# redradman/MujocoPoseLearning

Hardware: AMD Instinct MI355X
Metric: env steps/sec (whole node), humanoid 'stand' task, 1/2/4/8 MI355X (higher is better)
Workload: dtype f64

## Files before the change

### mujocoposelearning_amd/csrc/hs_contacts.h

```cpp
#pragma once
#include "hs_lanes.h"
#include "hs_scratch.h"

namespace hs {
namespace {

template <typename T>
struct Con {
  T pos[3], n[3], t1[3], dist;
};

template <typename T>
__device__ __forceinline__ bool plane_sphere(const T* pp, const T* pn, const T* c, T r, Con<T>& o) {
  T d[3] = {c[0] - pp[0], c[1] - pp[1], c[2] - pp[2]};
  T cd = dot3(d, pn);
  if (cd > r) return false;
  o.dist = cd - r;
  for (int k = 0; k < 3; k++) { o.n[k] = pn[k]; o.pos[k] = c[k] - pn[k] * (o.dist * T(0.5) + r); o.t1[k] = 0; }
  return true;
}
template <typename T>
__device__ __forceinline__ bool sphere_sphere(const T* p1, T r1, const T* p2, T r2, Con<T>& o) {
  T d[3] = {p2[0] - p1[0], p2[1] - p1[1], p2[2] - p1[2]};
  T len = sqrt(dot3(d, d));
// ... 56 lines not shown
  } else {
    T ax1[3] = {a1[0] * h1, a1[1] * h1, a1[2] * h1}, ax2[3] = {a2[0] * h2, a2[1] * h2, a2[2] * h2};
    T dif[3] = {p1[0] - p2[0], p1[1] - p2[1], p1[2] - p2[2]};
    T ma = dot3(ax1, ax1), mb = -dot3(ax1, ax2), mc = dot3(ax2, ax2), u = -dot3(ax1, dif), v = dot3(ax2, dif);
    T det = ma * mc - mb * mb;
    T v1[3], v2[3];
    if (fabs(det) >= T(1e-15)) {
      T x1 = (mc * u - mb * v) / det, x2 = (ma * v - mb * u) / det;
      if (x1 > 1) { x1 = 1; x2 = (v - mb) / mc; }
      else if (x1 < -1) { x1 = -1; x2 = (v + mb) / mc; }
      if (x2 > 1) { x2 = 1; x1 = (u - mb) / ma; x1 = x1 > 1 ? 1 : (x1 < -1 ? -1 : x1); }
      else if (x2 < -1) { x2 = -1; x1 = (u + mb) / ma; x1 = x1 > 1 ? 1 : (x1 < -1 ? -1 : x1); }
      for (int k = 0; k < 3; k++) { v1[k] = p1[k] + x1 * ax1[k]; v2[k] = p2[k] + x2 * ax2[k]; }
      n = sphere_sphere(v1, r1, v2, r2, c0) ? 1 : 0;
    } else {
      for (int side = 1; side >= -1; side -= 2) {
        T x2 = (v - side * mb) / mc;
        x2 = x2 > 1 ? 1 : (x2 < -1 ? -1 : x2);
        for (int k = 0; k < 3; k++) { v1[k] = p1[k] + side * ax1[k]; v2[k] = p2[k] + x2 * ax2[k]; }
        Con<T> t;
        if (sphere_sphere(v1, r1, v2, r2, t)) { if (n == 0) c0 = t; else c1 = t; n++; }
      }
    }
  }
  if (n > 0) make_frame(c0);
  if (n > 1) make_frame(c1);
  return n;
}

template <typename T, typename C>
__device__ __forceinline__ void store_contact(MPtr<T> m, Scratch<T, C>& s, int slot, const Con<T>& c, int p) {
  if (slot >= C::CON) return;
  for (int k = 0; k < 3; k++) { s.con_pos[slot][k] = c.pos[k]; s.con_n[slot][k] = c.n[k]; s.con_t1[slot][k] = c.t1[k]; }
  s.con_dist[slot] = c.dist;
  s.con_pair[slot] = p;
  const int b1 = m->pair_b1[p], b2 = m->pair_b2[p];
  s.con_bb[slot] = (uint32_t)b1 | (uint32_t)b2 << 8 | (uint32_t)m->pair_dim[p] << 16;
  s.con_m1[slot] = b1 ? HS_LT(C, m).body_chainmask[b1] : 0u;
  s.con_m2[slot] = HS_LT(C, m).body_chainmask[b2];
  s.con_mu[slot] = m->pair_mu[p];
}

static_assert(MAXPAIR <= 256 && MAXGEOM <= 256 && PAIR_CAPSULE_CAPSULE < 256, "near-pair entry: one byte per field");
__device__ __forceinline__ uint32_t near_entry(int p, int g1, int g2, int fn) {
  return (uint32_t)p | (uint32_t)g1 << 8 | (uint32_t)g2 << 16 | (uint32_t)fn << 24;
}
template <typename T, typename C>
__device__ __forceinline__ void store_contact_near(MPtr<T> m, Scratch<T, C>& s, int slot, const Con<T>& c, int p,
                                                   int g1, int g2, int dim, T mu) {
  if (slot >= C::CON) return;
  for (int k = 0; k < 3; k++) { s.con_pos[slot][k] = c.pos[k]; s.con_n[slot][k] = c.n[k]; s.con_t1[slot][k] = c.t1[k]; }
  s.con_dist[slot] = c.dist;
  s.con_pair[slot] = p;
  const int b1 = lanes<C>(m).geom_bodyid[g1], b2 = lanes<C>(m).geom_bodyid[g2];
  s.con_bb[slot] = (uint32_t)b1 | (uint32_t)b2 << 8 | (uint32_t)dim << 16;
  s.con_m1[slot] = b1 ? lanes<C>(m).body_chainmask[b1] : 0u;
  s.con_m2[slot] = lanes<C>(m).body_chainmask[b2];
  s.con_mu[slot] = mu;
}

template <typename T>
__device__ __forceinline__ T impedance(CPtr<T> si, T pos, T margin) {
  T s0 = fmin(T(0.9999), fmax(T(0.0001), si[0])), s1 = fmin(T(0.9999), fmax(T(0.0001), si[1]));
  if (s0 == s1 || si[2] <= T(1e-15)) return T(0.5) * (s0 + s1);
  T x = (pos - margin) * si[5];
  if (x < 0) x = -x;
  if (x >= 1 || x <= 0) return x >= 1 ? s1 : s0;
  const T p = si[4];
  T y = x;
  if (p != T(1)) {
    const bool lo = x <= si[3];
    const T base = lo ? x : 1 - x;
    T pw = base * base;
    if (p != T(2)) pw = pow(base, p);
    y = lo ? pw * si[6] : 1 - pw * si[7];
  }
  return s0 + y * (s1 - s0);
}

template <typename C, typename T>
__device__ __forceinline__ uint32_t chain_mask(MPtr<T> m, int sl, int nb) {
  return (sl > 0 && sl < nb) ? HS_LT(C, m).body_chainmask[sl] : 0u;
}
template <int NV, typename T, typename C>
__device__ __forceinline__ void map_vx(Scratch<T, C>& s, int sl, int nb, uint32_t ch) {
  if (sl < nb) {
    T v[6] = {0, 0, 0, 0, 0, 0};
    HS_FOR_BITS(C, G_VX, T)(ch, [&](int j) { ValsX<T, 6> r; r.x = s.vx[j]; for (int k = 0; k < 6; k++) r.v[k] = s.cdof[j][k]; return r; },
                [&](int, const ValsX<T, 6>& r) {
#pragma unroll
                  for (int k = 0; k < 6; k++) v[k] = fma(r.v[k], r.x, v[k]);
                });
    for (int k = 0; k < 6; k++) s.u.n.bvel[sl][k] = v[k];
  }
  WSYNC();
#pragma unroll
  for (int cs = 0; cs < C::CON; cs += HL) {
    const int c = cs + sl;
    if (c < s.ncon) {
      const uint32_t bb = s.con_bb[c];
      const int b1 = bb & 0xff, b2 = (bb >> 8) & 0xff;
      T r[3] = {s.con_pos[c][0] - s.com[0], s.con_pos[c][1] - s.com[1], s.con_pos[c][2] - s.com[2]};
      T w[3], v1[3], v2[3];
      cross3(s.u.n.bvel[b2], r, w);
      for (int k = 0; k < 3; k++) v2[k] = s.u.n.bvel[b2][3 + k] + w[k];
      cross3(s.u.n.bvel[b1], r, w);
      for (int k = 0; k < 3; k++) v1[k] = s.u.n.bvel[b1][3 + k] + w[k];
      T dv[3] = {v2[0] - v1[0], v2[1] - v1[1], v2[2] - v1[2]};
      T t2[3];
      cross3(s.con_n[c], s.con_t1[c], t2);
      s.con_v[c][0] = dot3(s.con_n[c], dv);
      s.con_v[c][1] = dot3(s.con_t1[c], dv);
      s.con_v[c][2] = dot3(t2, dv);
    }
  }
  WSYNC();
}

template <typename T, typename C>
__device__ __forceinline__ T row_Jx(MPtr<T> m, const Scratch<T, C>& s, int desc, T coef) {
  int kind = rk_kind(desc), j = rk_id(desc);
  if (kind <= RK_JHI) return coef * s.vx[j];
  if (kind <= RK_THI) {
    T v = 0;
    for (int w = 0; w < HS_LT(C, m).ten_nwrap[j]; w++) v += HS_LT(C, m).ten_wrapcoef[j][w] * s.vx[HS_LT(C, m).ten_wrapdof[j][w]];
    return coef * v;
  }
  int comp = kind == RK_CN ? 1 : 1 + ((kind - RK_P0) >> 1);
  return s.con_v[j][0] + coef * s.con_v[j][comp];
}

template <typename T, typename C>
__device__ __forceinline__ void row_u(MPtr<T> m, const Scratch<T, C>& s, int kind, int c, T* u) {
  if (kind == RK_CN) { for (int k = 0; k < 3; k++) u[k] = s.con_n[c][k]; return; }
  int sub = kind - RK_P0;
  T mu = s.con_mu[c];
  T sg = (sub & 1) ? -mu : mu;
  T t[3];
  if (sub >> 1) cross3(s.con_n[c], s.con_t1[c], t);
  else { t[0] = s.con_t1[c][0]; t[1] = s.con_t1[c][1]; t[2] = s.con_t1[c][2]; }
  for (int k = 0; k < 3; k++) u[k] = s.con_n[c][k] + sg * t[k];
}

template <typename T, typename C>
__device__ __forceinline__ void contact_aggregates(MPtr<T> m, Scratch<T, C>& s, int sl) {
  const bool up = threadIdx.x >= HL;
#pragma unroll
  for (int cs = 0; cs < C::CON; cs += HL) {
    const int c = cs + sl;
    bool act = false;
    if (c < s.ncon) {
      int adr = s.con_adr[c];
      int nr = (s.con_bb[c] >> 16) == 1 ? 1 : 4;
      T U[6] = {0, 0, 0, 0, 0, 0}, F[3] = {0, 0, 0};
      const bool pyr = nr == 4;
      T f4[4], D4[4], nn[3], t1[3], t2[3];
#pragma unroll
      for (int q = 0; q < 4; q++) {
        const bool on = q == 0 || pyr;
        f4[q] = on ? s.row_f[adr + q] : T(0);
        D4[q] = on ? s.row_D[adr + q] : T(0);
      }
      for (int k = 0; k < 3; k++) { nn[k] = s.con_n[c][k]; t1[k] = s.con_t1[c][k]; }
      const T mu = s.con_mu[c];
      cross3(nn, t1, t2);
#pragma unroll
      for (int q = 0; q < 4; q++) {
        const T f = f4[q];
        if (f != T(0)) {
          T u[3];
          if (!pyr) {
            for (int k = 0; k < 3; k++) u[k] = nn[k];
          } else {
            const T sg = (q & 1) ? -mu : mu;
            for (int k = 0; k < 3; k++) u[k] = nn[k] + sg * ((q >> 1) ? t2[k] : t1[k]);
          }
          const T D = D4[q];
          U[0] += D * u[0] * u[0]; U[1] += D * u[1] * u[1]; U[2] += D * u[2] * u[2];
          U[3] += D * u[0] * u[1]; U[4] += D * u[0] * u[2]; U[5] += D * u[1] * u[2];
          for (int k = 0; k < 3; k++) F[k] += f * u[k];
        }
      }
      for (int k = 0; k < 6; k++) s.con_U[c][k] = U[k];
      for (int k = 0; k < 3; k++) s.con_F[c][k] = F[k];
      act = F[0] != T(0) || F[1] != T(0) || F[2] != T(0) || U[0] != T(0) || U[1] != T(0) || U[2] != T(0);
    }
    const uint32_t mk = hballot(act, up);
    if (sl == 0) s.con_act[cs / HL] = mk;
  }
  WSYNC();
}
template <typename C, typename F>
__device__ __forceinline__ void for_active_contacts(const uint32_t* act, F&& f) {
#pragma unroll
  for (int w = 0; w < (C::CON + HL - 1) / HL; w++)
    for (uint32_t mk = act[w]; mk; mk &= mk - 1u) f(w * HL + __builtin_ctz(mk));
}

template <typename T, typename C, typename LD, typename F>
__device__ __forceinline__ void for_active_contacts_ld(const uint32_t* act, LD&& ld, F&& f) {
#pragma unroll
  for (int w = 0; w < (C::CON + HL - 1) / HL; w++)
    for_bits<T, true>(
        act[w], [&](int j) { return ld(w * HL + j); }, [&](int j, const auto& v) { f(w * HL + j, v); });
}

template <typename T, typename C>
__device__ __forceinline__ T jtf_lane(MPtr<T> m, const Scratch<T, C>& s, int sl, const T* cd) {
  T acc = 0;
  struct CV { uint32_t m1, m2; T p[3], f[3]; };
  for_active_contacts_ld<T, C>(s.con_act, [&](int c) {
    CV v;
    v.m1 = s.con_m1[c]; v.m2 = s.con_m2[c];
    for (int k = 0; k < 3; k++) { v.p[k] = s.con_pos[c][k]; v.f[k] = s.con_F[c][k]; }
    return v;
  }, [&](int, const CV& v) {
    const int in2 = bit(v.m2, sl), in1 = bit(v.m1, sl);
    if (in1 != in2) {
      T r[3] = {v.p[0] - s.com[0], v.p[1] - s.com[1], v.p[2] - s.com[2]};
      T w[3];
      cross3(cd, r, w);
      T jp[3] = {cd[3] + w[0], cd[4] + w[1], cd[5] + w[2]};
      T x = dot3(jp, v.f);
      acc += in2 ? x : -x;
    }
  });
  if (sl < MAXDOF) {
    int lr = s.lim_row[sl];
    int lo = (lr & 0xff) - 1, hi = (lr >> 8) - 1;
    if (lo >= 0) acc += s.row_f[lo];
    if (hi >= 0) acc -= s.row_f[hi];
  }
  for (int r = s.njl; r < s.nlim; r++) {
    int id = rk_id(s.row_kid[r]);
    T f = rk_kind(s.row_kid[r]) == RK_TLO ? s.row_f[r] : -s.row_f[r];
    for (int w = 0; w < HS_LT(C, m).ten_nwrap[id]; w++)
      if (HS_LT(C, m).ten_wrapdof[id][w] == sl) acc += f * HS_LT(C, m).ten_wrapcoef[id][w];
  }
  return acc;
}

}
}
```

### mujocoposelearning_amd/csrc/hs_env_step.h

```cpp
#pragma once
#include <cmath>
#include <cstdint>

#include "hs_philox.h"
#include "hs_stepper.h"
#include "hs_reward.h"
#include "hs_policy.h"
#include "hs_term_builtin.h"

namespace hs {
namespace {

__device__ __forceinline__ uint64_t splitmix(uint64_t x) {
  x += 0x9E3779B97F4A7C15ull;
  x = (x ^ (x >> 30)) * 0xBF58476D1CE4E5B9ull;
  x = (x ^ (x >> 27)) * 0x94D049BB133111EBull;
  return x ^ (x >> 31);
}
template <typename T>
__device__ __forceinline__ T uniform_pm(uint64_t seed, int env, uint32_t episode, int k, T scale) {
  uint64_t h = splitmix(seed ^ splitmix(((uint64_t)env << 32) ^ ((uint64_t)episode << 8) ^ (uint64_t)k));
  double u = (double)(h >> 11) * (1.0 / 9007199254740992.0);
  return (T)(-scale + 2.0 * scale * u);
}

template <typename T, typename C>
__device__ __forceinline__ void reset_state(MPtr<T> m, Scratch<T, C>& s, int sl, T& time, T& xws) {
  if (sl < m->nq) s.qpos[sl] = m->qpos0[sl];
  if (sl + HL < m->nq) s.qpos[sl + HL] = m->qpos0[sl + HL];
  if (sl < m->nv) s.qvel[sl] = 0;
  if (sl < m->nu) s.ctrl[sl] = 0;
  xws = 0;
  time = 0;
  WSYNC();
}

template <typename T, int NV, bool PGS, typename C>
__device__ __forceinline__ void physics_step(Stepper<T, NV, C>& st, KPtr<T> k, T& time, T& xws, int* warn,
                                             PgsCache<T, C>* pc) {
  MPtr<T> m = st.m;
  Scratch<T, C>& s = st.s;
  const int sl = st.sl;
  const bool up = st.up;
  bool bq = (sl < m->nq && isbad(s.qpos[sl])) || (sl + HL < m->nq && isbad(s.qpos[sl + HL]));
  bool bv = sl < m->nv && isbad(s.qvel[sl]);
  if (hballot(bq, up)) { warn[WARN_BADQPOS]++; reset_state(m, s, sl, time, xws); }
  else if (hballot(bv, up)) { warn[WARN_BADQVEL]++; reset_state(m, s, sl, time, xws); }
  T D[C::RPL], ar[C::RPL], rc[C::RPL];
  int rd[C::RPL];
  for (int attempt = 0; attempt < 2; attempt++) {
    HS_STAMP(st.clk, 0);
    st.kinematics();
    HS_STAMP(st.clk, 1);
    if constexpr (C::NEAR) {
      if (st.collision_near()) warn[WARN_OVERFLOW]++;
    } else {
      if (st.collision()) warn[WARN_OVERFLOW]++;
    }
    HS_STAMP(st.clk, 4);
    st.mass_matrix();
    HS_STAMP(st.clk, 2);
    st.velocity_forces();
    HS_STAMP(st.clk, 3);
    if (st.rows(D, ar, rd, rc)) warn[WARN_OVERFLOW]++;
    HS_STAMP(st.clk, 5);
    if constexpr (PGS)
      st.solve_pgs(xws, opaque(k)->p.max_newton, D, ar, rd, rc, *pc);
    else
      st.solve(xws, opaque(k)->p.max_newton, sizeof(T) == 8 ? T(1e-13) : T(1e-7), D, ar, rd, rc);
    bool ba = sl < m->nv && isbad(st.qacc);
    bool redo = hballot(ba, up) != 0 && attempt == 0;
    if (__ballot(redo) == 0) break;
    if (redo) {
      warn[WARN_BADQACC]++;
      reset_state(m, s, sl, time, xws);
    }
  }
  if (opaque(k)->p.full_state) st.post_constraint();
  st.euler(time);
  HS_STAMP(st.clk, 13);
  xws = st.qacc;
}

template <bool UC = false, typename T, typename C, typename O>
__device__ __forceinline__ void write_obs(MPtr<T> m, const Scratch<T, C>& s, int sl, T qfa, O* out,
                          int obs_dim) {
  auto put = [&](int i, O v) {
    if constexpr (UC) row_st(out + i, v);
    else out[i] = v;
  };
  int nq = m->nq, nv = m->nv;
  int o1 = nq - 2, o2 = o1 + nv, o3 = o2 + 10 * m->nbody, o4 = o3 + 6 * m->nbody;
  for (int k = sl; k < o4; k += HL) {
    T v;
    if (k < o1) v = s.qpos[2 + k];
    else if (k < o2) v = s.qvel[k - o1];
    else if (k < o3) { int q = k - o2; v = s.cinert[q / 10][q % 10]; }
    else { int q = k - o3; v = s.cvel[q / 6][q % 6]; }
    put(k, (O)v);
  }
  if (sl < nv && o4 + sl < obs_dim) put(o4 + sl, (O)qfa);
  const int o5 = o4 + nv, nf = 6 * (m->nbody - 1);
  if (obs_dim >= o5 + nf)
    for (int k = sl; k < nf; k += HL) put(o5 + k, (O)s.u.n.cfrc[1 + k / 6][k % 6]);
}

template <typename T, int NV, typename C>
__device__ __forceinline__ void dump_debug(const Stepper<T, NV, C>& st, T* dbg) {
  const Scratch<T, C>& s = st.s;
  int sl = st.sl;
  for (int k = sl; k < MAXBODY * 10; k += HL) dbg[200 + k] = s.cinert[k / 10][k % 10];
  for (int k = sl; k < MAXDOF * 6; k += HL) dbg[500 + k] = s.cdof[k / 6][k % 6];
  if (sl < NV)
    for (int j = 0; j < NV; j++) dbg[700 + sl * MAXDOF + j] = st.Mr[j];
  for (int k = sl; k < MAXBODY * 6; k += HL) dbg[1800 + k] = s.cvel[k / 6][k % 6];
  if (sl < NV) {
    dbg[2280 + sl] = st.qfa;
    dbg[2320 + sl] = st.fsmooth;
    dbg[2360 + sl] = st.fcon;
    dbg[2400 + sl] = st.qacc;
  }
  if (sl == 0) {
    dbg[2500] = s.com[0]; dbg[2501] = s.com[1]; dbg[2502] = s.com[2];
    dbg[2503] = s.ncon; dbg[2504] = s.nefc; dbg[2505] = st.niter; dbg[2506] = s.nlim;
  }
  for (int c = sl; c < s.ncon; c += HL) {
    T* o = dbg + 2600 + 11 * c;
    for (int k = 0; k < 3; k++) { o[k] = s.con_pos[c][k]; o[3 + k] = s.con_n[c][k]; o[6 + k] = s.con_t1[c][k]; }
    o[9] = s.con_dist[c];
    o[10] = s.con_pair[c];
  }
  for (int r = sl; r < s.nefc; r += HL) {
    T* o = dbg + 4000 + 6 * r;
    o[0] = rk_kind(s.row_kid[r]); o[1] = rk_id(s.row_kid[r]); o[2] = s.row_D[r]; o[4] = s.row_f[r];
  }
}

template <typename T, int NV, typename C>
__device__ __forceinline__ void commit(MPtr<T> m, KPtr<T> k, const Stepper<T, NV, C>& st,
                       int env, T time, T xws, int step_count, uint32_t episode, T total, const int* warn,
                       bool full) {
  const Scratch<T, C>& s = st.s;
  const int sl = st.sl, nq = m->nq, nv = m->nv, nu = m->nu;
  const int outputs = k->p.outputs;
  if (sl < nq) k->b.qpos[(size_t)env * nq + sl] = s.qpos[sl];
  if (sl + HL < nq) k->b.qpos[(size_t)env * nq + sl + HL] = s.qpos[sl + HL];
  if (sl < nv) {
    k->b.qvel[(size_t)env * nv + sl] = s.qvel[sl];
    k->b.qacc_ws[(size_t)env * nv + sl] = xws;
    if (outputs & OUT_AUX) k->b.aux[(size_t)env * AUXDIM + sl] = st.qacc;
  }
  if (sl < nu && ((outputs & OUT_CTRL) || k->p.mode != MODE_ENV_STEP)) k->b.ctrl[(size_t)env * nu + sl] = s.ctrl[sl];
// ... 486 lines not shown
```

### mujocoposelearning_amd/csrc/hs_lanes.h

```cpp
#pragma once
#include <hip/hip_runtime.h>

#include <cstdint>
#include <type_traits>

#include "hs_kernels.h"
#include "hs_model.h"
#include "hs_bits.h"

namespace hs {
namespace {

constexpr int WAVE = 64;
constexpr int HL = 32;
static_assert(MAXDOF == HL, "one dof per sub-lane (lim_row slots, dof masks)");

template <int NCON, int NEFC, bool W = false, bool LT = false>
struct Cap {
  static constexpr int CON = NCON;
  static constexpr int EFC = NEFC;
  static constexpr int RPL = NEFC / HL;
  static constexpr bool WIDE = W;
  static constexpr bool LANES = LT;
  static constexpr bool NEAR = LT;
  static constexpr bool GROUPS = LT;
  static_assert((NCON % HL == 0 || HL % NCON == 0) && NEFC % HL == 0, "capacity in whole half-waves");
};
template <typename T>
using Resident = std::conditional_t<sizeof(T) == 8, Cap<MAXCON_F64, MAXEFC_F64, false, true>, Cap<MAXCON, MAXEFC>>;
using Wide = Cap<MAXCON_WIDE, MAXEFC_WIDE, true>;

#define SCHED_FENCE() __builtin_amdgcn_sched_barrier(0)

#define WSYNC() asm volatile("" ::: "memory")

template <int B, int E, typename F>
__device__ __forceinline__ void static_for(F&& f) {
  if constexpr (B < E) {
    f(std::integral_constant<int, B>{});
    static_for<B + 1, E>(f);
  }
}
template <int CTRL>
__device__ __forceinline__ uint32_t dpp32(uint32_t v) {
  return (uint32_t)__builtin_amdgcn_mov_dpp((int)v, CTRL, 0xF, 0xF, true);
}
struct RowPair { uint32_t lo, hi; };
__device__ __forceinline__ RowPair rowswap(uint32_t v) {
  auto r = __builtin_amdgcn_permlane16_swap(v, v, false, false);
  return {r[0], r[1]};
}
template <int K>
__device__ __forceinline__ uint32_t bcast32(uint32_t v) {
  RowPair r = rowswap(dpp32<0x150 + (K & 15)>(v));
  return K < 16 ? r.lo : r.hi;
}
template <int K>
__device__ __forceinline__ float bcast(float v) {
  return __uint_as_float(bcast32<K>(__float_as_uint(v)));
}
template <int K>
__device__ __forceinline__ double bcast(double v) {
  uint64_t x = (uint64_t)__double_as_longlong(v);
  uint64_t lo = bcast32<K>((uint32_t)x), hi = bcast32<K>((uint32_t)(x >> 32));
  return __longlong_as_double((long long)((hi << 32) | lo));
}
template <int CTRL>
__device__ __forceinline__ float dpp(float v) {
  return __uint_as_float(dpp32<CTRL>(__float_as_uint(v)));
}
template <int CTRL>
__device__ __forceinline__ double dpp(double v) {
  uint64_t x = (uint64_t)__double_as_longlong(v);
  uint64_t lo = dpp32<CTRL>((uint32_t)x), hi = dpp32<CTRL>((uint32_t)(x >> 32));
  return __longlong_as_double((long long)((hi << 32) | lo));
}
__device__ __forceinline__ float rows_sum(float v) {
  RowPair r = rowswap(__float_as_uint(v));
  return __uint_as_float(r.lo) + __uint_as_float(r.hi);
}
__device__ __forceinline__ double rows_sum(double v) {
  uint64_t x = (uint64_t)__double_as_longlong(v);
  RowPair l = rowswap((uint32_t)x), h = rowswap((uint32_t)(x >> 32));
  return __longlong_as_double((long long)(((uint64_t)h.lo << 32) | l.lo)) +
         __longlong_as_double((long long)(((uint64_t)h.hi << 32) | l.hi));
}
__device__ __forceinline__ float up_row(float v) { return __uint_as_float(rowswap(__float_as_uint(v)).hi); }
__device__ __forceinline__ double up_row(double v) {
  uint64_t x = (uint64_t)__double_as_longlong(v);
  const uint64_t lo = rowswap((uint32_t)x).hi, hi = rowswap((uint32_t)(x >> 32)).hi;
  return __longlong_as_double((long long)((hi << 32) | lo));
}
template <typename T>
__device__ __forceinline__ T hsum(T v) {
  v += dpp<0xB1>(v);
  v += dpp<0x4E>(v);
  v += dpp<0x141>(v);
  v += dpp<0x140>(v);
  return rows_sum(v);
}
__device__ __forceinline__ uint32_t hballot(bool p, bool upper) {
  uint64_t m = __ballot(p);
  return upper ? (uint32_t)(m >> 32) : (uint32_t)m;
}
template <typename T, bool AHEAD = false, typename LD, typename F>
__device__ __forceinline__ void for_bits(uint32_t mk, LD&& ld, F&& f) {
  if constexpr (AHEAD) {
    if (mk == 0u) return;
// ... 223 lines not shown
```

### mujocoposelearning_amd/csrc/hs_stepper.h

```cpp
#pragma once
#include "hs_contacts.h"
#include "hs_dense.h"
#include "hs_lanes.h"
#include "hs_phase_clock.h"
#include "hs_scratch.h"

namespace hs {
namespace {

template <typename T, int NV, typename C>
struct Stepper {
  PhaseClock clk;
  MPtr<T> m;
  Scratch<T, C>& s;
  int sl, nb;
  bool up;
  T cd[6];
  T Mr[NV];
  T fsmooth;
  T fcon;
  T qacc;
  T qfa;
  T damp;
  int niter;
// ... 298 lines not shown
      anci = HS_LT(C, m).dof_ancmask[sl];
      arm = HS_LT(C, m).dof_armature[sl];
    }
    WSYNC();
    {
      T cb2[2][12];
      auto load = [&](auto jc, T (&dst)[12]) {
        constexpr int j = decltype(jc)::value;
        for (int k = 0; k < 6; k++) { dst[k] = s.cdof[j][k]; dst[6 + k] = s.u.c.buf[j][k]; }
      };
      load(std::integral_constant<int, 0>{}, cb2[0]);
      static_for<0, NV>([&](auto jc) {
        constexpr int j = decltype(jc)::value;
        if constexpr (j + 1 < NV) load(std::integral_constant<int, j + 1>{}, cb2[(j + 1) & 1]);
        SCHED_FENCE();
        const uint32_t ancj = m->dof_ancmask[j];
        const bool rel = (sl < NV) && (bit(anci, j) || bit(ancj, sl));
        const T* cj = cb2[j & 1];
        const T v = (j <= sl) ? dot6(cj, bf) : dot6(cd, cj + 6);
        Mr[j] = rel ? v + ((j == sl) ? arm : T(0)) : T(0);
      });
    }
    WSYNC();
  }

  __device__ __forceinline__ void velocity_forces() {
    phase_begin();
    if (sl < nb) {
      T v[6] = {0, 0, 0, 0, 0, 0};
      if (sl > 0) {
        const uint32_t ch = HS_LT(C, m).body_chainmask[sl];
        HS_FOR_BITS(C, G_VEL, T)(ch, [&](int j) { ValsX<T, 6> r; r.x = s.qvel[j]; for (int k = 0; k < 6; k++) r.v[k] = s.cdof[j][k]; return r; },
                    [&](int, const ValsX<T, 6>& r) { for (int k = 0; k < 6; k++) v[k] = fma(r.v[k], r.x, v[k]); });
      }
      for (int k = 0; k < 6; k++) s.cvel[sl][k] = v[k];
    }
    if (sl < NV) {
      const uint32_t dm = HS_LT(C, m).dof_dotmask[sl];
      T v[6] = {0, 0, 0, 0, 0, 0}, cdd[6];
      HS_FOR_BITS(C, G_VEL, T)(dm, [&](int j) { ValsX<T, 6> r; r.x = s.qvel[j]; for (int k = 0; k < 6; k++) r.v[k] = s.cdof[j][k]; return r; },
                  [&](int, const ValsX<T, 6>& r) { for (int k = 0; k < 6; k++) v[k] = fma(r.v[k], r.x, v[k]); });
      cross_motion(v, cd, cdd);
      for (int k = 0; k < 6; k++) s.u.r.cdofdot[sl][k] = cdd[k];
    }
    WSYNC();
    if (sl > 0 && sl < nb) {
      const uint32_t ch = HS_LT(C, m).body_chainmask[sl];
      T a[6] = {0, 0, 0, -m->gravity[0], -m->gravity[1], -m->gravity[2]};
      HS_FOR_BITS(C, G_VEL, T)(ch, [&](int j) { ValsX<T, 6> r; r.x = s.qvel[j]; for (int k = 0; k < 6; k++) r.v[k] = s.u.r.cdofdot[j][k]; return r; },
                  [&](int, const ValsX<T, 6>& r) { for (int k = 0; k < 6; k++) a[k] = fma(r.v[k], r.x, a[k]); });
      T f[6], t[6], t2[6];
      mul_inert(s.cinert[sl], a, f);
      mul_inert(s.cinert[sl], s.cvel[sl], t);
      cross_force(s.cvel[sl], t, t2);
      for (int k = 0; k < 6; k++) s.u.r.cfrc[sl][k] = f[k] + t2[k];
    }
    WSYNC();
    if (sl > 0 && sl < nb) {
      const uint32_t dm = HS_LT(C, m).body_descmask[sl] & ~1u & ((nb < 32 ? (1u << nb) : 0u) - 1u);
      T a[6] = {0, 0, 0, 0, 0, 0};
      HS_FOR_BITS(C, G_VEL, T)(dm, [&](int c) { Vals<T, 6> r; for (int k = 0; k < 6; k++) r.v[k] = s.u.r.cfrc[c][k]; return r; },
                  [&](int, const Vals<T, 6>& r) { for (int k = 0; k < 6; k++) a[k] += r.v[k]; });
      for (int k = 0; k < 6; k++) s.u.r.csub[sl][k] = a[k];
    }
    WSYNC();
    fsmooth = 0;
    qfa = 0;
    if (sl < NV) {
      T bias = dot6(cd, s.u.r.csub[HS_LT(C, m).dof_bodyid[sl]]);
      int qa = HS_LT(C, m).dof_qposadr[sl];
      T pas = -HS_LT(C, m).dof_damping[sl] * s.qvel[sl];
      if (qa >= 0) pas -= HS_LT(C, m).dof_stiffness[sl] * (s.qpos[qa] - HS_LT(C, m).dof_springref[sl]);
      int u = HS_LT(C, m).dof_actuator[sl];
      if (u >= 0) {
        T c = s.ctrl[u];
        if (HS_LT(C, m).act_ctrllimited[u]) c = fmin(HS_LT(C, m).act_ctrlrange[u][1], fmax(HS_LT(C, m).act_ctrlrange[u][0], c));
        qfa = HS_LT(C, m).act_gear[u] * c;
      }
      fsmooth = pas - bias + qfa;
    }
    WSYNC();
  }

  __device__ __forceinline__ int rows(T (&D)[C::RPL], T (&ar)[C::RPL], int (&rd)[C::RPL], T (&rc)[C::RPL]) {
    phase_begin();
    damp = sl < NV ? HS_LT(C, m).dof_damping[sl] : T(0);
    int overflow = 0;
    int ncon = s.ncon;
    int nrow = 0;
    {
      bool lo = false, hi = false;
      if (sl < m->njnt && HS_LT(C, m).jnt_limited[sl]) {
        T q = s.qpos[HS_LT(C, m).jnt_qposadr[sl]];
        lo = (q - HS_LT(C, m).jnt_range[sl][0]) < HS_LT(C, m).jnt_margin[sl];
        hi = (HS_LT(C, m).jnt_range[sl][1] - q) < HS_LT(C, m).jnt_margin[sl];
      }
      uint32_t ml = hballot(lo, up), mh = hballot(hi, up);
      int pre = below(ml, sl) + below(mh, sl);
      if (lo) s.row_kid[pre] = (RK_JLO << 16) | sl;
      if (hi) s.row_kid[pre + lo] = (RK_JHI << 16) | sl;
      nrow = __popc(ml) + __popc(mh);
      s.lim_row[sl] = 0;
      if (lo || hi)
        s.lim_row[HS_LT(C, m).jnt_dofadr[sl]] = (uint16_t)((lo ? pre + 1 : 0) | (hi ? (pre + lo + 1) << 8 : 0));
    }
    const int njl = nrow;
    {
      bool lo = false, hi = false;
      if (sl < m->ntendon && HS_LT(C, m).ten_limited[sl]) {
        T L = 0;
        for (int w = 0; w < HS_LT(C, m).ten_nwrap[sl]; w++) L += HS_LT(C, m).ten_wrapcoef[sl][w] * s.qpos[HS_LT(C, m).ten_wrapqadr[sl][w]];
        lo = (L - HS_LT(C, m).ten_range[sl][0]) < m->ten_margin[sl];
        hi = (HS_LT(C, m).ten_range[sl][1] - L) < m->ten_margin[sl];
      }
      uint32_t ml = hballot(lo, up), mh = hballot(hi, up);
      int pre = nrow + below(ml, sl) + below(mh, sl);
      if (lo) s.row_kid[pre] = (RK_TLO << 16) | sl;
      if (hi) s.row_kid[pre + lo] = (RK_THI << 16) | sl;
      nrow += __popc(ml) + __popc(mh);
    }
    int nlim = nrow;
    {
      int tot = 0;
#pragma unroll
      for (int cs = 0; cs < C::CON; cs += HL) {
        const int c = cs + sl;
        const bool isc = c < ncon;
        const bool pyr = isc && (s.con_bb[c] >> 16) == 3;
        tot += __popc(hballot(isc, up)) + 3 * __popc(hballot(pyr, up));
      }
      if (nrow + tot > C::EFC) {
        overflow = 1;
        int fit = 0, nr = nrow;
        for (int c = 0; c < ncon; c++) {
          int need = (s.con_bb[c] >> 16) == 3 ? 4 : 1;
          if (nr + need > C::EFC) break;
          nr += need;
          fit++;
        }
        ncon = fit;
      }
#pragma unroll
      for (int cs = 0; cs < C::CON; cs += HL) {
        const int c = cs + sl;
        const bool isc = c < ncon;
        const bool pyr = isc && (s.con_bb[c] >> 16) == 3;
        const uint32_t mc = hballot(isc, up), mp = hballot(pyr, up);
        const int pre = nrow + below(mc, sl) + 3 * below(mp, sl);
        if (isc) {
          s.con_adr[c] = pre;
          if (!pyr) s.row_kid[pre] = (RK_CN << 16) | c;
          else for (int q = 0; q < 4; q++) s.row_kid[pre + q] = ((RK_P0 + q) << 16) | c;
        }
        nrow += __popc(mc) + 3 * __popc(mp);
      }
    }
    if (sl == 0) { s.ncon = ncon; s.nefc = nrow; s.nlim = nlim; s.njl = njl; }
    if (sl < NV) s.vx[sl] = s.qvel[sl];
    WSYNC();
    map_vx<NV>(s, sl, nb, chain_mask<C>(m, sl, nb));
#pragma unroll
    for (int q = 0; q < C::RPL; q++) {
      int r = sl + HL * q;
      D[q] = 0;
      ar[q] = 0;
      rd[q] = 0;
      rc[q] = 0;
      bool dense = false;
      if (r < nrow) {
        int kid = s.row_kid[r];
        int kind = rk_kind(kid), id = rk_id(kid);
        T pos, margin, dA, rscale = 1;
        CPtr<T> sr;
        CPtr<T> si;
        if (kind <= RK_JHI) {
          T qv = s.qpos[HS_LT(C, m).jnt_qposadr[id]];
          pos = kind == RK_JLO ? qv - HS_LT(C, m).jnt_range[id][0] : HS_LT(C, m).jnt_range[id][1] - qv;
          margin = HS_LT(C, m).jnt_margin[id];
          sr = m->jnt_solref[id]; si = m->jnt_solimp[id];
          int dof = HS_LT(C, m).jnt_dofadr[id];
          dA = HS_LT(C, m).dof_invweight0[dof];
          rd[q] = (kind << 16) | dof;
          rc[q] = kind == RK_JLO ? T(1) : T(-1);
        } else if (kind <= RK_THI) {
          T L = 0;
          for (int w = 0; w < HS_LT(C, m).ten_nwrap[id]; w++) L += HS_LT(C, m).ten_wrapcoef[id][w] * s.qpos[HS_LT(C, m).ten_wrapqadr[id][w]];
          pos = kind == RK_TLO ? L - HS_LT(C, m).ten_range[id][0] : HS_LT(C, m).ten_range[id][1] - L;
          margin = m->ten_margin[id];
          sr = m->ten_solref[id]; si = m->ten_solimp[id];
          dA = m->ten_invweight0[id];
          rd[q] = kid;
          rc[q] = kind == RK_TLO ? T(1) : T(-1);
          dense = true;
        } else {
          int p = s.con_pair[id];
          pos = s.con_dist[id];
          margin = m->pair_margin[p];
          sr = m->pair_solref[p]; si = m->pair_solimp[p];
          const uint32_t bb = s.con_bb[id];
          T tran = HS_LT(C, m).body_invweight_tran[bb & 0xff] + HS_LT(C, m).body_invweight_tran[(bb >> 8) & 0xff];
          T mu = s.con_mu[id];
          dA = kind == RK_CN ? tran : tran + mu * mu * tran;
          if (kind != RK_CN) rscale = 2 * mu * mu;
          rd[q] = kid;
          rc[q] = kind == RK_CN ? T(0) : (((kind - RK_P0) & 1) ? -mu : mu);
          dense = s.con_m1[id] != 0u;
        }
        T imp = impedance(si, pos, margin);
        T dmax = fmin(T(0.9999), fmax(T(0.0001), si[1]));
        T K, B;
        if (sr[0] > 0) {
          T tc = fmax(sr[0], 2 * m->timestep), dr = sr[1];
          const T u = recip(dmax * tc), ud = u * recip(dr);
          K = ud * ud;
          B = 2 * u;
        } else {
          const T v = recip(dmax);
          K = -sr[0] * v * v;
          B = -sr[1] * v;
        }
        T R = rscale * fmax(T(1e-15), (1 - imp) * dA * recip(imp));
        D[q] = recip(R);
        s.row_D[r] = D[q];
        ar[q] = -B * row_Jx(m, s, rd[q], rc[q]) - K * imp * (pos - margin);
      }
      uint32_t dm = hballot(dense, up);
      if (sl == 0) s.dense_mask[q] = dm;
    }
    WSYNC();
    return overflow;
  }

  __device__ __forceinline__ void solve(T xws, int maxit, T tol, const T (&D)[C::RPL], const T (&ar)[C::RPL],
                                        const int (&rd)[C::RPL], const T (&rc)[C::RPL]) {
    phase_begin();
    const int nefc = s.nefc;
    T x = sl < NV ? xws : T(0);
    bool vr[C::RPL];
#pragma unroll
    for (int q = 0; q < C::RPL; q++) vr[q] = sl + HL * q < nefc;
    const uint32_t anci = sl < NV ? HS_LT(C, m).dof_ancmask[sl] : 0u;
    const uint32_t bch = chain_mask<C>(m, sl, nb);
    const T scale = m->newton_scale;
    if (sl < NV) s.vx[sl] = x;
    WSYNC();
    T Mx = matvec_lds(Mr, s.vx);
    map_vx<NV>(s, sl, nb, bch);
    T jar[C::RPL], Js[C::RPL];
#pragma unroll
    for (int q = 0; q < C::RPL; q++) jar[q] = vr[q] ? row_Jx(m, s, rd[q], rc[q]) - ar[q] : T(0);
    HS_STAMP(clk, 6);
    bool done = false;
    int it = 0;
    if (sl == 0) s.niter = maxit;
    for (; it < maxit; it++) {
      m = opaque(m);
      sl = opaque_v(sl);
      bool act[C::RPL];
#pragma unroll
      for (int q = 0; q < C::RPL; q++) {
        act[q] = vr[q] && jar[q] < 0;
        if (vr[q]) s.row_f[sl + HL * q] = act[q] ? -D[q] * jar[q] : T(0);
      }
      WSYNC();
      contact_aggregates(m, s, sl);
      HS_STAMP(clk, 7);
      T jtf = jtf_lane(m, s, sl, cd);
      T g = sl < NV ? Mx - fsmooth - jtf : T(0);
      const T gn2 = hsum(g * g);
      const bool conv = scale * scale * gn2 < tol * tol;
      if (conv && !done && sl == 0) s.niter = it;
      done = done || conv;
      HS_STAMP(clk, 8);
      if (__ballot(!done) == 0) break;
      T H[NV];
      T hdinv = 0, hdiag = 0;
      {
        T aug[6] = {0, 0, 0, 0, 0, 0};
        T dadd = 0;
        struct CU { uint32_t m1, m2; T p[3], U[6]; };
        for_active_contacts_ld<T, C>(s.con_act, [&](int c) {
          CU v;
          v.m1 = s.con_m1[c]; v.m2 = s.con_m2[c];
          for (int k = 0; k < 3; k++) v.p[k] = s.con_pos[c][k];
          for (int k = 0; k < 6; k++) v.U[k] = s.con_U[c][k];
          return v;
        }, [&](int, const CU& v) {
          if (v.m1 != 0u || !bit(v.m2, sl)) return;
          T r[3] = {v.p[0] - s.com[0], v.p[1] - s.com[1], v.p[2] - s.com[2]};
          T w[3];
          cross3(cd, r, w);
          T jp[3] = {cd[3] + w[0], cd[4] + w[1], cd[5] + w[2]};
          const T* U = v.U;
          T z[3] = {U[0] * jp[0] + U[3] * jp[1] + U[4] * jp[2], U[3] * jp[0] + U[1] * jp[1] + U[5] * jp[2],
                    U[4] * jp[0] + U[5] * jp[1] + U[2] * jp[2]};
          T rz[3];
          cross3(r, z, rz);
          for (int k = 0; k < 3; k++) { aug[k] += rz[k]; aug[3 + k] += z[k]; }
        });
        {
          int lr = s.lim_row[sl];
          int lo = (lr & 0xff) - 1, hi = (lr >> 8) - 1;
          if (lo >= 0 && s.row_f[lo] != T(0)) dadd += s.row_D[lo];
          if (hi >= 0 && s.row_f[hi] != T(0)) dadd += s.row_D[hi];
        }
        HS_STAMP(clk, 27);
        constexpr int HESS_G = sizeof(T) == 8 ? 2 : 1;
        if constexpr (HESS_G == 1) {
#pragma unroll
          for (int j = 0; j < NV; j++) {
            T cj[6];
            for (int k = 0; k < 6; k++) cj[k] = s.cdof[j][k];
            H[j] = Mr[j] + (bit(anci, j) ? dot6(cj, aug) : T(0)) + ((j == sl) ? dadd : T(0));
            SCHED_FENCE();
          }
        } else {
          constexpr int NG = (NV + HESS_G - 1) / HESS_G;
          T cbuf[2][HESS_G][6];
          auto load = [&](auto gc, T (&dst)[HESS_G][6]) {
            constexpr int j0 = decltype(gc)::value * HESS_G;
            static_for<0, HESS_G>([&](auto tc) {
              constexpr int t = decltype(tc)::value;
              if constexpr (j0 + t < NV)
                for (int k = 0; k < 6; k++) dst[t][k] = s.cdof[j0 + t][k];
            });
          };
          load(std::integral_constant<int, 0>{}, cbuf[0]);
          static_for<0, NG>([&](auto gc) {
            constexpr int g = decltype(gc)::value, j0 = g * HESS_G;
            if constexpr (g + 1 < NG) load(std::integral_constant<int, g + 1>{}, cbuf[(g + 1) & 1]);
            SCHED_FENCE();
            static_for<0, HESS_G>([&](auto tc) {
              constexpr int t = decltype(tc)::value, j = j0 + t;
              if constexpr (j < NV)
                H[j] = Mr[j] + (bit(anci, j) ? dot6(cbuf[g & 1][t], aug) : T(0)) + ((j == sl) ? dadd : T(0));
            });
          });
        }
        HS_STAMP(clk, 28);
        uint32_t dm[C::RPL];
#pragma unroll
        for (int q = 0; q < C::RPL; q++) dm[q] = s.dense_mask[q] & hballot(act[q], up);
        for (;;) {
          int r = -1;
#pragma unroll
          for (int q = C::RPL - 1; q >= 0; q--)
            if (dm[q]) r = HL * q + __builtin_ctz(dm[q]);
          if (__ballot(r >= 0) == 0) break;
          T jr = 0, Dr = 0;
          if (r >= 0) {
            dm[r / HL] &= dm[r / HL] - 1u;
            if (s.row_f[r] != T(0)) {
              int kid = s.row_kid[r];
              int kind = rk_kind(kid), id = rk_id(kid);
              Dr = s.row_D[r];
              if (kind == RK_TLO || kind == RK_THI) {
                for (int w = 0; w < HS_LT(C, m).ten_nwrap[id]; w++)
                  if (HS_LT(C, m).ten_wrapdof[id][w] == sl) jr += HS_LT(C, m).ten_wrapcoef[id][w];
                if (kind == RK_THI) jr = -jr;
              } else {
                int in2 = bit(s.con_m2[id], sl), in1 = bit(s.con_m1[id], sl);
                if (in1 != in2) {
                  T rr[3] = {s.con_pos[id][0] - s.com[0], s.con_pos[id][1] - s.com[1], s.con_pos[id][2] - s.com[2]};
                  T w[3], u[3];
                  cross3(cd, rr, w);
                  T jp[3] = {cd[3] + w[0], cd[4] + w[1], cd[5] + w[2]};
                  row_u(m, s, kind, id, u);
                  jr = in2 ? dot3(u, jp) : -dot3(u, jp);
                }
              }
            }
          }
          if (sl >= NV) jr = 0;
          T dj = Dr * jr;
          static_for<0, NV>([&](auto jc) {
            constexpr int j = decltype(jc)::value;
            H[j] += dj * bcast<j>(jr);
          });
        }
      }
      HS_STAMP(clk, 9);
      chol_rows<NV, T, LDLF>(H, hdinv, sl, s.u.n.cb, &hdiag);
      HS_STAMP(clk, 15);
      T sdir = -chol_solve<NV, T, LDLF>(H, hdinv, g, sl);
      if (sl >= NV) sdir = 0;
      HS_STAMP(clk, 10);
      if (sl < NV) s.vx[sl] = sdir;
      WSYNC();
      T Ms = matvec_lds(Mr, s.vx);
      T A0 = hsum(sl < NV ? sdir * Ms : T(0));
      T B0 = hsum(sl < NV ? sdir * (Mx - fsmooth) : T(0));
      HS_STAMP(clk, 18);
      map_vx<NV>(s, sl, nb, bch);
      HS_STAMP(clk, 19);
#pragma unroll
      for (int q = 0; q < C::RPL; q++) Js[q] = vr[q] ? row_Jx(m, s, rd[q], rc[q]) : T(0);
      HS_STAMP(clk, 16);
      bool same1 = true;
#pragma unroll
      for (int q = 0; q < C::RPL; q++) same1 = same1 && (!vr[q] || ((jar[q] + Js[q] < 0) == act[q]));
      bool lsdone = done || (hballot(!same1, up) == 0);
      T alpha = 1, lo = 0, hi = T(1e30);
      T d0 = 0;
      {
        T c = 0;
#pragma unroll
        for (int q = 0; q < C::RPL; q++) c += act[q] ? D[q] * jar[q] * Js[q] : T(0);
        d0 = B0 + hsum(c);
      }
      const T ltol = (sizeof(T) == 8 ? T(1e-10) : T(1e-5)) * fabs(d0);
      for (int ls = 0; ls < 30; ls++) {
        if (__ballot(!lsdone) == 0) break;
        T c1 = 0, c2 = 0;
#pragma unroll
        for (int q = 0; q < C::RPL; q++) {
          T jq = jar[q] + alpha * Js[q];
          bool a = vr[q] && jq < 0;
          c1 += a ? D[q] * jq * Js[q] : T(0);
          c2 += a ? D[q] * Js[q] * Js[q] : T(0);
        }
        T d1 = B0 + alpha * A0 + hsum(c1);
        T d2 = A0 + hsum(c2);
        if (!lsdone) {
          if (fabs(d1) <= ltol) {
            lsdone = true;
          } else {
            if (d1 < 0) lo = alpha; else hi = alpha;
            T an = d2 > 0 ? alpha - d1 * recip(d2) : T(-1);
            if (!(an > lo && an < hi)) an = hi < T(1e29) ? T(0.5) * (lo + hi) : T(2) * alpha;
            if (hi - lo <= (sizeof(T) == 8 ? T(1e-14) : T(1e-6)) * hi) lsdone = true;
            else alpha = an;
          }
        }
      }
      HS_STAMP(clk, 11);
      if (!done) {
        x += alpha * sdir;
        Mx += alpha * Ms;
        bool changed = false;
#pragma unroll
        for (int q = 0; q < C::RPL; q++) {
          T nj = jar[q] + alpha * Js[q];
          changed = changed || (vr[q] && ((nj < 0) != act[q]));
          jar[q] = nj;
        }
        if (hballot(changed, up) == 0 && fabs(alpha - T(1)) < T(1e-3)) {
          done = true;
          if (sl == 0) s.niter = it + 1;
        }
      }
      if (__ballot(!done) == 0) { it++; break; }
    }
    WSYNC();
    niter = s.niter;
#pragma unroll
    for (int q = 0; q < C::RPL; q++)
      if (vr[q]) s.row_f[sl + HL * q] = jar[q] < 0 ? -D[q] * jar[q] : T(0);
    WSYNC();
    contact_aggregates(m, s, sl);
    fcon = sl < NV ? jtf_lane(m, s, sl, cd) : T(0);
    qacc = x;
    WSYNC();
    HS_STAMP(clk, 12);
  }

  __device__ __forceinline__ T row_J_lane(int r) {
    if (sl >= NV) return T(0);
    const int kid = s.row_kid[r];
    const int kind = rk_kind(kid), id = rk_id(kid);
    if (kind <= RK_JHI) return HS_LT(C, m).jnt_dofadr[id] == sl ? (kind == RK_JLO ? T(1) : T(-1)) : T(0);
    if (kind <= RK_THI) {
      T v = 0;
      for (int w = 0; w < HS_LT(C, m).ten_nwrap[id]; w++)
        if (HS_LT(C, m).ten_wrapdof[id][w] == sl) v += HS_LT(C, m).ten_wrapcoef[id][w];
      return kind == RK_TLO ? v : -v;
    }
    const int in2 = bit(s.con_m2[id], sl), in1 = bit(s.con_m1[id], sl);
    if (in1 == in2) return T(0);
    T rr[3] = {s.con_pos[id][0] - s.com[0], s.con_pos[id][1] - s.com[1], s.con_pos[id][2] - s.com[2]};
// ... 272 lines not shown
```

Before: 6.963 million.

## Fuse constraint row velocity walks and merge Hessian augmentation into jtf pass

During row building, the Newton path now computes chain velocities for qvel and the warm-start vector in one pass over the kinematic chain. It derives the initial Jacobian-times-x values from that pass, so the solver no longer needs its own map_vx pass before iterating. Inside the Newton loop, the contact Hessian augmentation is folded into the same active-contact walk that computes J^T f, removing a second traversal. Row Jacobian products are batched with loads issued up front and a ballot-guarded tendon path. In exchange, register pressure rises and the code becomes harder to follow.

```diff
diff --git a/mujocoposelearning_amd/csrc/hs_contacts.h b/mujocoposelearning_amd/csrc/hs_contacts.h
--- a/mujocoposelearning_amd/csrc/hs_contacts.h
+++ b/mujocoposelearning_amd/csrc/hs_contacts.h
@@ -162,18 +162,8 @@
 __device__ __forceinline__ uint32_t chain_mask(MPtr<T> m, int sl, int nb) {
   return (sl > 0 && sl < nb) ? HS_LT(C, m).body_chainmask[sl] : 0u;
 }
-template <int NV, typename T, typename C>
-__device__ __forceinline__ void map_vx(Scratch<T, C>& s, int sl, int nb, uint32_t ch) {
-  if (sl < nb) {
-    T v[6] = {0, 0, 0, 0, 0, 0};
-    HS_FOR_BITS(C, G_VX, T)(ch, [&](int j) { ValsX<T, 6> r; r.x = s.vx[j]; for (int k = 0; k < 6; k++) r.v[k] = s.cdof[j][k]; return r; },
-                [&](int, const ValsX<T, 6>& r) {
-#pragma unroll
-                  for (int k = 0; k < 6; k++) v[k] = fma(r.v[k], r.x, v[k]);
-                });
-    for (int k = 0; k < 6; k++) s.u.n.bvel[sl][k] = v[k];
-  }
-  WSYNC();
+template <typename T, typename C>
+__device__ __forceinline__ void contact_vel(Scratch<T, C>& s, int sl, const T (*bv)[6]) {
 #pragma unroll
   for (int cs = 0; cs < C::CON; cs += HL) {
     const int c = cs + sl;
@@ -182,10 +172,10 @@
       const int b1 = bb & 0xff, b2 = (bb >> 8) & 0xff;
       T r[3] = {s.con_pos[c][0] - s.com[0], s.con_pos[c][1] - s.com[1], s.con_pos[c][2] - s.com[2]};
       T w[3], v1[3], v2[3];
-      cross3(s.u.n.bvel[b2], r, w);
-      for (int k = 0; k < 3; k++) v2[k] = s.u.n.bvel[b2][3 + k] + w[k];
-      cross3(s.u.n.bvel[b1], r, w);
-      for (int k = 0; k < 3; k++) v1[k] = s.u.n.bvel[b1][3 + k] + w[k];
+      cross3(bv[b2], r, w);
+      for (int k = 0; k < 3; k++) v2[k] = bv[b2][3 + k] + w[k];
+      cross3(bv[b1], r, w);
+      for (int k = 0; k < 3; k++) v1[k] = bv[b1][3 + k] + w[k];
       T dv[3] = {v2[0] - v1[0], v2[1] - v1[1], v2[2] - v1[2]};
       T t2[3];
       cross3(s.con_n[c], s.con_t1[c], t2);
@@ -193,6 +183,34 @@
       s.con_v[c][1] = dot3(s.con_t1[c], dv);
       s.con_v[c][2] = dot3(t2, dv);
     }
+  }
+  WSYNC();
+}
+template <int NV, typename T, typename C>
+__device__ __forceinline__ void map_vx(Scratch<T, C>& s, int sl, int nb, uint32_t ch) {
+  if (sl < nb) {
+    T v[6] = {0, 0, 0, 0, 0, 0};
+    HS_FOR_BITS(C, G_VX, T)(ch, [&](int j) { ValsX<T, 6> r; r.x = s.vx[j]; for (int k = 0; k < 6; k++) r.v[k] = s.cdof[j][k]; return r; },
+                [&](int, const ValsX<T, 6>& r) {
+#pragma unroll
+                  for (int k = 0; k < 6; k++) v[k] = fma(r.v[k], r.x, v[k]);
+                });
+    for (int k = 0; k < 6; k++) s.u.n.bvel[sl][k] = v[k];
+  }
+  WSYNC();
+  contact_vel(s, sl, s.u.n.bvel);
+}
+template <int NV, typename T, typename C>
+__device__ __forceinline__ void chain_vel2(Scratch<T, C>& s, int sl, int nb, uint32_t ch) {
+  struct V2 { T x, y; T v[6]; };
+  if (sl < nb) {
+    T v[6] = {0, 0, 0, 0, 0, 0}, u[6] = {0, 0, 0, 0, 0, 0};
+    for_bits_g<C, G_VX, T>(ch, [&](int j) { V2 r; r.x = s.qvel[j]; r.y = s.vx[j]; for (int k = 0; k < 6; k++) r.v[k] = s.cdof[j][k]; return r; },
+                           [&](int, const V2& r) {
+#pragma unroll
+                             for (int k = 0; k < 6; k++) { v[k] = fma(r.v[k], r.x, v[k]); u[k] = fma(r.v[k], r.y, u[k]); }
+                           });
+    for (int k = 0; k < 6; k++) { s.u.n.bvel[sl][k] = v[k]; s.u.n.cfrc[sl][k] = u[k]; }
   }
   WSYNC();
 }
@@ -208,6 +226,41 @@
   }
   int comp = kind == RK_CN ? 1 : 1 + ((kind - RK_P0) >> 1);
   return s.con_v[j][0] + coef * s.con_v[j][comp];
+}
+
+template <typename T, typename C>
+__device__ __forceinline__ void rows_Jx(MPtr<T> m, const Scratch<T, C>& s, const T* xv, const bool (&vr)[C::RPL],
+                                        const int (&rd)[C::RPL], const T (&rc)[C::RPL], T (&out)[C::RPL]) {
+  T a[C::RPL], b[C::RPL];
+  bool ten = false;
+#pragma unroll
+  for (int q = 0; q < C::RPL; q++) {
+    const int kind = rk_kind(rd[q]), j = rk_id(rd[q]);
+    const bool con = kind >= RK_CN;
+    const int comp = kind == RK_CN ? 1 : 1 + ((kind - RK_P0) >> 1);
+    const T* p0 = con ? &s.con_v[j][0] : &xv[j];
+    const T* p1 = con ? &s.con_v[j][comp] : p0;
+    a[q] = *p0;
+    b[q] = *p1;
+    ten = ten || (vr[q] && kind >= RK_TLO && kind <= RK_THI);
+  }
+  SCHED_FENCE();
+#pragma unroll
+  for (int q = 0; q < C::RPL; q++) {
+    const T cv = fma(rc[q], b[q], a[q]), jv = rc[q] * a[q];
+    out[q] = vr[q] ? (rk_kind(rd[q]) >= RK_CN ? cv : jv) : T(0);
+  }
+  if (__ballot(ten) != 0) {
+#pragma unroll
+    for (int q = 0; q < C::RPL; q++) {
+      const int kind = rk_kind(rd[q]), j = rk_id(rd[q]);
+      if (vr[q] && kind >= RK_TLO && kind <= RK_THI) {
+        T v = 0;
+        for (int w = 0; w < HS_LT(C, m).ten_nwrap[j]; w++) v += HS_LT(C, m).ten_wrapcoef[j][w] * xv[HS_LT(C, m).ten_wrapdof[j][w]];
+        out[q] = rc[q] * v;
+      }
+    }
+  }
 }
 
 template <typename T, typename C>
@@ -286,13 +339,36 @@
 }
 
 template <typename T, typename C>
-__device__ __forceinline__ T jtf_lane(MPtr<T> m, const Scratch<T, C>& s, int sl, const T* cd) {
+__device__ __forceinline__ T jtf_tail(MPtr<T> m, const Scratch<T, C>& s, int sl, T acc) {
+  if (sl < MAXDOF) {
+    int lr = s.lim_row[sl];
+    int lo = (lr & 0xff) - 1, hi = (lr >> 8) - 1;
+    if (lo >= 0) acc += s.row_f[lo];
+    if (hi >= 0) acc -= s.row_f[hi];
+  }
+  for (int r = s.njl; r < s.nlim; r++) {
+    int id = rk_id(s.row_kid[r]);
+    T f = rk_kind(s.row_kid[r]) == RK_TLO ? s.row_f[r] : -s.row_f[r];
+    for (int w = 0; w < HS_LT(C, m).ten_nwrap[id]; w++)
+      if (HS_LT(C, m).ten_wrapdof[id][w] == sl) acc += f * HS_LT(C, m).ten_wrapcoef[id][w];
+  }
+  return acc;
+}
+
+template <typename T>
+struct ConF { uint32_t m1, m2; T p[3], f[3]; };
+template <typename T>
+struct ConFU { uint32_t m1, m2; T p[3], f[3], U[6]; };
+template <bool AUG, typename T, typename C>
+__device__ __forceinline__ T jtf_walk(MPtr<T> m, const Scratch<T, C>& s, int sl, const T* cd, T* aug) {
   T acc = 0;
-  struct CV { uint32_t m1, m2; T p[3], f[3]; };
+  using CV = std::conditional_t<AUG, ConFU<T>, ConF<T>>;
   for_active_contacts_ld<T, C>(s.con_act, [&](int c) {
     CV v;
     v.m1 = s.con_m1[c]; v.m2 = s.con_m2[c];
     for (int k = 0; k < 3; k++) { v.p[k] = s.con_pos[c][k]; v.f[k] = s.con_F[c][k]; }
+    if constexpr (AUG)
+      for (int k = 0; k < 6; k++) v.U[k] = s.con_U[c][k];
     return v;
   }, [&](int, const CV& v) {
     const int in2 = bit(v.m2, sl), in1 = bit(v.m1, sl);
@@ -303,22 +379,28 @@
       T jp[3] = {cd[3] + w[0], cd[4] + w[1], cd[5] + w[2]};
       T x = dot3(jp, v.f);
       acc += in2 ? x : -x;
+      if constexpr (AUG) {
+        if (v.m1 == 0u) {
+          const T* U = v.U;
+          T z[3] = {U[0] * jp[0] + U[3] * jp[1] + U[4] * jp[2], U[3] * jp[0] + U[1] * jp[1] + U[5] * jp[2],
+                    U[4] * jp[0] + U[5] * jp[1] + U[2] * jp[2]};
+          T rz[3];
+          cross3(r, z, rz);
+          for (int k = 0; k < 3; k++) { aug[k] += rz[k]; aug[3 + k] += z[k]; }
+        }
+      }
     }
   });
-  if (sl < MAXDOF) {
-    int lr = s.lim_row[sl];
-    int lo = (lr & 0xff) - 1, hi = (lr >> 8) - 1;
-    if (lo >= 0) acc += s.row_f[lo];
-    if (hi >= 0) acc -= s.row_f[hi];
-  }
-  for (int r = s.njl; r < s.nlim; r++) {
-    int id = rk_id(s.row_kid[r]);
-    T f = rk_kind(s.row_kid[r]) == RK_TLO ? s.row_f[r] : -s.row_f[r];
-    for (int w = 0; w < HS_LT(C, m).ten_nwrap[id]; w++)
-      if (HS_LT(C, m).ten_wrapdof[id][w] == sl) acc += f * HS_LT(C, m).ten_wrapcoef[id][w];
-  }
-  return acc;
-}
-
-}
-}
+  return jtf_tail(m, s, sl, acc);
+}
+template <typename T, typename C>
+__device__ __forceinline__ T jtf_lane(MPtr<T> m, const Scratch<T, C>& s, int sl, const T* cd) {
+  return jtf_walk<false>(m, s, sl, cd, (T*)nullptr);
+}
+template <typename T, typename C>
+__device__ __forceinline__ T jtf_aug_lane(MPtr<T> m, const Scratch<T, C>& s, int sl, const T* cd, T (&aug)[6]) {
+  return jtf_walk<true>(m, s, sl, cd, aug);
+}
+
+}
+}
diff --git a/mujocoposelearning_amd/csrc/hs_env_step.h b/mujocoposelearning_amd/csrc/hs_env_step.h
--- a/mujocoposelearning_amd/csrc/hs_env_step.h
+++ b/mujocoposelearning_amd/csrc/hs_env_step.h
@@ -46,7 +46,7 @@
   bool bv = sl < m->nv && isbad(s.qvel[sl]);
   if (hballot(bq, up)) { warn[WARN_BADQPOS]++; reset_state(m, s, sl, time, xws); }
   else if (hballot(bv, up)) { warn[WARN_BADQVEL]++; reset_state(m, s, sl, time, xws); }
-  T D[C::RPL], ar[C::RPL], rc[C::RPL];
+  T D[C::RPL], ar[C::RPL], rc[C::RPL], jar0[C::RPL];
   int rd[C::RPL];
   for (int attempt = 0; attempt < 2; attempt++) {
     HS_STAMP(st.clk, 0);
@@ -62,12 +62,12 @@
     HS_STAMP(st.clk, 2);
     st.velocity_forces();
     HS_STAMP(st.clk, 3);
-    if (st.rows(D, ar, rd, rc)) warn[WARN_OVERFLOW]++;
+    if (st.template rows<!PGS>(D, ar, rd, rc, xws, jar0)) warn[WARN_OVERFLOW]++;
     HS_STAMP(st.clk, 5);
     if constexpr (PGS)
       st.solve_pgs(xws, opaque(k)->p.max_newton, D, ar, rd, rc, *pc);
     else
-      st.solve(xws, opaque(k)->p.max_newton, sizeof(T) == 8 ? T(1e-13) : T(1e-7), D, ar, rd, rc);
+      st.solve(xws, opaque(k)->p.max_newton, sizeof(T) == 8 ? T(1e-13) : T(1e-7), D, ar, rd, rc, jar0);
     bool ba = sl < m->nv && isbad(st.qacc);
     bool redo = hballot(ba, up) != 0 && attempt == 0;
     if (__ballot(redo) == 0) break;
diff --git a/mujocoposelearning_amd/csrc/hs_lanes.h b/mujocoposelearning_amd/csrc/hs_lanes.h
--- a/mujocoposelearning_amd/csrc/hs_lanes.h
+++ b/mujocoposelearning_amd/csrc/hs_lanes.h
@@ -24,6 +24,7 @@
   static constexpr bool LANES = LT;
   static constexpr bool NEAR = LT;
   static constexpr bool GROUPS = LT;
+  static constexpr bool WALKS = LT;
   static_assert((NCON % HL == 0 || HL % NCON == 0) && NEFC % HL == 0, "capacity in whole half-waves");
 };
 template <typename T>
diff --git a/mujocoposelearning_amd/csrc/hs_stepper.h b/mujocoposelearning_amd/csrc/hs_stepper.h
--- a/mujocoposelearning_amd/csrc/hs_stepper.h
+++ b/mujocoposelearning_amd/csrc/hs_stepper.h
@@ -404,7 +404,10 @@
     WSYNC();
   }
 
-  __device__ __forceinline__ int rows(T (&D)[C::RPL], T (&ar)[C::RPL], int (&rd)[C::RPL], T (&rc)[C::RPL]) {
+  template <bool NEWTON>
+  __device__ __forceinline__ int rows(T (&D)[C::RPL], T (&ar)[C::RPL], int (&rd)[C::RPL], T (&rc)[C::RPL], T xws,
+                                      T (&jar0)[C::RPL]) {
+    constexpr bool WK = C::WALKS && NEWTON;
     phase_begin();
     damp = sl < NV ? HS_LT(C, m).dof_damping[sl] : T(0);
     int overflow = 0;
@@ -478,13 +481,22 @@
       }
     }
     if (sl == 0) { s.ncon = ncon; s.nefc = nrow; s.nlim = nlim; s.njl = njl; }
-    if (sl < NV) s.vx[sl] = s.qvel[sl];
-    WSYNC();
-    map_vx<NV>(s, sl, nb, chain_mask<C>(m, sl, nb));
+    if constexpr (WK) {
+      if (sl < NV) s.vx[sl] = xws;
+      WSYNC();
+      chain_vel2<NV>(s, sl, nb, chain_mask<C>(m, sl, nb));
+      contact_vel(s, sl, s.u.n.bvel);
+    } else {
+      if (sl < NV) s.vx[sl] = s.qvel[sl];
+      WSYNC();
+      map_vx<NV>(s, sl, nb, chain_mask<C>(m, sl, nb));
+    }
+    [[maybe_unused]] T rB[WK ? C::RPL : 1], rKi[WK ? C::RPL : 1], rpm[WK ? C::RPL : 1];
 #pragma unroll
     for (int q = 0; q < C::RPL; q++) {
       int r = sl + HL * q;
       D[q] = 0;
+      if constexpr (WK) { rB[q] = 0; rKi[q] = 0; rpm[q] = 0; }
       ar[q] = 0;
       rd[q] = 0;
       rc[q] = 0;
@@ -544,17 +556,34 @@
         T R = rscale * fmax(T(1e-15), (1 - imp) * dA * recip(imp));
         D[q] = recip(R);
         s.row_D[r] = D[q];
-        ar[q] = -B * row_Jx(m, s, rd[q], rc[q]) - K * imp * (pos - margin);
+        if constexpr (WK) { rB[q] = B; rKi[q] = K * imp; rpm[q] = pos - margin; }
+        else ar[q] = -B * row_Jx(m, s, rd[q], rc[q]) - K * imp * (pos - margin);
       }
       uint32_t dm = hballot(dense, up);
       if (sl == 0) s.dense_mask[q] = dm;
     }
+    if constexpr (WK) {
+      bool vr[C::RPL];
+      T jx[C::RPL];
+#pragma unroll
+      for (int q = 0; q < C::RPL; q++) vr[q] = sl + HL * q < nrow;
+      rows_Jx(m, s, s.qvel, vr, rd, rc, jx);
+#pragma unroll
+      for (int q = 0; q < C::RPL; q++)
+        if (vr[q]) ar[q] = -rB[q] * jx[q] - rKi[q] * rpm[q];
+      WSYNC();
+      contact_vel(s, sl, s.u.n.cfrc);
+      rows_Jx(m, s, s.vx, vr, rd, rc, jx);
+#pragma unroll
+      for (int q = 0; q < C::RPL; q++) jar0[q] = vr[q] ? jx[q] - ar[q] : T(0);
+    }
     WSYNC();
     return overflow;
   }
 
   __device__ __forceinline__ void solve(T xws, int maxit, T tol, const T (&D)[C::RPL], const T (&ar)[C::RPL],
-                                        const int (&rd)[C::RPL], const T (&rc)[C::RPL]) {
+                                        const int (&rd)[C::RPL], const T (&rc)[C::RPL], const T (&jar0)[C::RPL]) {
+    constexpr bool WK = C::WALKS;
     phase_begin();
     const int nefc = s.nefc;
     T x = sl < NV ? xws : T(0);
@@ -567,10 +596,15 @@
     if (sl < NV) s.vx[sl] = x;
     WSYNC();
     T Mx = matvec_lds(Mr, s.vx);
-    map_vx<NV>(s, sl, nb, bch);
     T jar[C::RPL], Js[C::RPL];
-#pragma unroll
-    for (int q = 0; q < C::RPL; q++) jar[q] = vr[q] ? row_Jx(m, s, rd[q], rc[q]) - ar[q] : T(0);
+    if constexpr (WK) {
+#pragma unroll
+      for (int q = 0; q < C::RPL; q++) jar[q] = jar0[q];
+    } else {
+      map_vx<NV>(s, sl, nb, bch);
+#pragma unroll
+      for (int q = 0; q < C::RPL; q++) jar[q] = vr[q] ? row_Jx(m, s, rd[q], rc[q]) - ar[q] : T(0);
+    }
     HS_STAMP(clk, 6);
     bool done = false;
     int it = 0;
@@ -587,7 +621,10 @@
       WSYNC();
       contact_aggregates(m, s, sl);
       HS_STAMP(clk, 7);
-      T jtf = jtf_lane(m, s, sl, cd);
+      T aug[6] = {0, 0, 0, 0, 0, 0};
+      T jtf;
+      if constexpr (WK) jtf = jtf_aug_lane(m, s, sl, cd, aug);
+      else jtf = jtf_lane(m, s, sl, cd);
       T g = sl < NV ? Mx - fsmooth - jtf : T(0);
       const T gn2 = hsum(g * g);
       const bool conv = scale * scale * gn2 < tol * tol;
@@ -598,10 +635,9 @@
       T H[NV];
       T hdinv = 0, hdiag = 0;
       {
-        T aug[6] = {0, 0, 0, 0, 0, 0};
         T dadd = 0;
         struct CU { uint32_t m1, m2; T p[3], U[6]; };
-        for_active_contacts_ld<T, C>(s.con_act, [&](int c) {
+        if constexpr (!WK) for_active_contacts_ld<T, C>(s.con_act, [&](int c) {
           CU v;
           v.m1 = s.con_m1[c]; v.m2 = s.con_m2[c];
           for (int k = 0; k < 3; k++) v.p[k] = s.con_pos[c][k];
@@ -715,8 +751,12 @@
       HS_STAMP(clk, 18);
       map_vx<NV>(s, sl, nb, bch);
       HS_STAMP(clk, 19);
-#pragma unroll
-      for (int q = 0; q < C::RPL; q++) Js[q] = vr[q] ? row_Jx(m, s, rd[q], rc[q]) : T(0);
+      if constexpr (WK) {
+        rows_Jx(m, s, s.vx, vr, rd, rc, Js);
+      } else {
+#pragma unroll
+        for (int q = 0; q < C::RPL; q++) Js[q] = vr[q] ? row_Jx(m, s, rd[q], rc[q]) : T(0);
+      }
       HS_STAMP(clk, 16);
       bool same1 = true;
 #pragma unroll
```

Measured after the change: 7.143 million (median of 6 runs). +2.6%, better.
